# B-R-P/NMSLIB-ZIG

Measured on AMD Instinct MI355X. Metric: queries/sec @ recall@10, 1M x 128-D L2, batch=1024; HBM GB/s vs peak, higher is better.
Workload: dtype f16+f32

## Files before the change

nmslib_zig_amd/csrc/brute.cpp:

```cpp
#include <algorithm>
#include <cmath>
#include <cstdlib>
#include <cstring>

#include "engine.hpp"
#include "l1_quant.hpp"

namespace gfxknn {

void BruteDense::release() {
    have_bf16 = false;
    have_l1 = false;
    l1_u8.release();
    l1_cols.release();
    bf_hi.release();
    bf_lo.release();
    f16_hi.release();
    auxp.release();
    auxp16.release();
}

size_t BruteDense::bytes() const {
    size_t total = 0;
    for (const DevBuf* b : {&rows_i8, &auxh, &rows_sel, &mean, &bf_hi, &bf_lo, &auxp, &f16_hi, &auxp16, &l1_u8, &l1_cols}) total += b->bytes();
// ... 228 lines not shown
    auto fast_ws = [&](const BfFastWsBytes& need) {
        BfFastWs ws{};
        ws.top8 = b.ws_top8.ensure(need.top8);
        ws.thr = b.ws_thr.ensure(need.thr);
        ws.list = static_cast<uint32_t*>(b.ws_list.ensure(need.list));
        ws.list_cnt = static_cast<int*>(b.ws_listcnt.ensure(need.list_cnt));
        ws.fb.cand = static_cast<unsigned long long*>(ws_cand_.ensure(need.cand));
        ws.fb.cnt = static_cast<int*>(ws_cnt_.ensure(need.cnt));
        if (need.flags_fb) ws.flags_fb = static_cast<int*>(b.ws_flags.ensure(need.flags_fb));
        if (need.queries) ws.queries = b.ws_f32_q.ensure(need.queries);
        return ws;
    };
    if (is_u8()) {
        const BfU8Fast f = bf_u8_fast_plan((int)d_n_, (int)nq, (int)k);
        if (f.use) {
            ws_qpad_.ensure((size_t)f.qpad * 128);
            const BfFastWs ws = fast_ws(bf_fast_ws_bytes(f));
            const BfU8Rows rows{d_rows_.as<uint8_t>(), b.rows_i8.as<uint8_t>(), d_aux_.as<int32_t>(), b.auxh.as<int32_t>(), (int)d_n_};
            hip_check(launch_bf_u8_fast(f, (int)nq, (int)k, rows, static_cast<const uint8_t*>(d_queries), ws_qpad_.as<uint8_t>(),
                                        ws, out, prof_pair(), stream),
                      "bf_u8_fast");
            last_path = 3;
            fast_flags_ = ws.tile_fail(f);
            fast_nqt_ = f.nqt;
            fast_has_precise_ = false;
            return;
        }
    }
    const BfF32Rows rows{d_rows_.as<float>(), b.centred ? b.rows_sel.as<float>() : d_rows_.as<float>(), d_aux_.as<float>(),
                         (int)d_n_, dim_eff, d_n_ ? ldb_ : f32_row_stride(dim_eff), b.bmax};
    BfF32Queries q{};
    if (!is_u8() && b.have_bf16) {
        const BfF32Fast f = bf_f32_fast_plan((int)d_n_, dim_eff, (int)nq, (int)k, space_, b.centred);
        if (f.use) {
            const int ldb = ldb_;
            q.padded = static_cast<float*>(ws_qpad_.ensure((size_t)f.qpad * ldb * 4));
            q.sel = q.padded;
            q.scale_q = b.f16_scale_q;
            if (b.centred) {
                hip_check(launch_pad_rows(d_queries, (int)nq, dim_eff, q.padded, f.qpad, ldb, 4, stream), "pad queries");
                ws_qsel_.ensure((size_t)f.qpad * ldb * 4);
                hip_check(launch_center_rows(q.padded, b.mean.as<float>(), f.qpad, (int)nq, ldb, dim_eff, ws_qsel_.as<float>(),
                                             stream),
                          "centre queries");
                q.sel = ws_qsel_.as<float>();
            } else {
                q.raw = static_cast<const float*>(d_queries);
            }
            if (f.cosc) {
                ws_qaux_.ensure((size_t)f.qpad * 16);
                b.ws_qaug.ensure((size_t)f.qpad * f.dp * 4);
                q.centred = ws_qsel_.as<float>();
                q.qaux_cosc = ws_qaux_.as<float>();
                hip_check(launch_query_aux_cosc(q.padded, q.centred, f.qpad, ldb, dim_eff, b.mu_norm, ws_qaux_.as<float>(), stream),
                          "query aux");
                hip_check(launch_query_aug_cosc(q.centred, q.qaux_cosc, (int)nq, f.qpad, ldb, dim_eff, b.cosc_lambda,
                                                b.ws_qaug.as<float>(), f.dp, stream),
                          "augmented queries");
                q.sel = b.ws_qaug.as<float>();
                q.sel_ld = f.dp;
            }
            const BfFastWs ws = fast_ws(bf_fast_ws_bytes(f));
            hip_check(launch_bf_f32_fast(f, space_, (int)nq, (int)k, rows, b.tiles(f.dp, f.cosc), q, ws, out, prof_pair(), stream),
                      "bf_f32_fast");
            last_path = 1;
            fast_flags_ = ws.tile_fail(f);
            fast_nqt_ = f.nqt;
            fast_has_precise_ = true;
            return;
        }
    }
    if (space_ == SP_L1 && b.have_l1) {
        const char* env = getenv("NMSLIB_GPU_L1_FAST");
        const BfL1Fast f = bf_l1_fast_plan((int)d_n_, dim_eff, (int)nq, (int)k);
        if (f.use && !(env && atoi(env) == 0)) {
            ws_qpad_.ensure((size_t)f.qpad * ldb_ * 4);
            BfL1Ws ws{};
            ws.qt = static_cast<uint32_t*>(b.ws_l1_qt.ensure((size_t)f.d4 * f.qpad * 4));
            ws.xe = static_cast<double*>(b.ws_l1_xe.ensure((size_t)f.qpad * 16));
            ws.cand.cand = static_cast<unsigned long long*>(b.ws_l1_cand.ensure((size_t)f.qpad * f.nsplit * f.kprime * 8));
            ws.cand.cnt = static_cast<int*>(b.ws_l1_cnt.ensure((size_t)f.qpad * f.nsplit * 4));
            ws.flags = static_cast<int*>(b.ws_flags.ensure((size_t)f.nqt * 4 + 64));
            ws.fb.cand = static_cast<unsigned long long*>(ws_cand_.ensure(bf_cand_elems(f.fallback) * 8));
            ws.fb.cnt = static_cast<int*>(ws_cnt_.ensure(bf_cnt_elems(f.fallback) * 4));
            const float* cols = b.l1_cols.as<float>();
            const BfL1Rows copy{b.l1_u8.as<uint32_t>(), cols, cols + dim_, cols + 2 * dim_, b.l1_step};
            hip_check(launch_bf_l1_fast(f, (int)nq, (int)k, rows, copy, static_cast<const float*>(d_queries), ws_qpad_.as<float>(),
                                        ws, out, prof_pair(), stream),
                      "bf_l1_fast");
            last_path = 6;
            fast_flags_ = ws.flags;
            fast_nqt_ = f.nqt;
            fast_has_precise_ = false;
            return;
        }
    }
    last_path = is_u8() ? 2 : 0;
    BfPlan p = bf_make_plan((int)d_n_, dim_eff, (int)nq, (int)k, is_u8());
    if (d_n_ == 0) p.ldb = is_u8() ? 128 : f32_row_stride(dim_eff);
    const int elem = is_u8() ? 1 : 4;
    ws_qpad_.ensure((size_t)p.qpad * p.ldb * elem);
    const BfCand c{static_cast<unsigned long long*>(ws_cand_.ensure(bf_cand_elems(p) * 8)),
                   static_cast<int*>(ws_cnt_.ensure(bf_cnt_elems(p) * 4))};
    hip_check(launch_pad_rows(d_queries, (int)nq, dim_eff, ws_qpad_.ptr(), p.qpad, p.ldb, elem, stream), "pad queries");
    q.padded = ws_qpad_.as<float>();
    q.sel = q.padded;
    if (b.centred) {
        ws_qsel_.ensure((size_t)p.qpad * p.ldb * 4);
        hip_check(launch_center_rows(q.padded, b.mean.as<float>(), p.qpad, (int)nq, p.ldb, dim_eff, ws_qsel_.as<float>(), stream),
                  "centre queries");
        q.sel = ws_qsel_.as<float>();
        if (space_ != SP_L2) {
            ws_qaux_.ensure((size_t)p.qpad * 16);
            hip_check(launch_query_aux_cosc(q.padded, q.sel, p.qpad, p.ldb, dim_eff, b.mu_norm, ws_qaux_.as<float>(), stream),
// ... 24 lines not shown
```

nmslib_zig_amd/csrc/engine.cpp:

```cpp
#include "engine.hpp"
#include "f16_pack.hpp"

#include <algorithm>
#include <chrono>
#include <cmath>
#include <cstring>
#include <fstream>
#include <set>
#include <sstream>
#include <thread>

namespace gfxknn {

using clk = std::chrono::steady_clock;

void hip_check(hipError_t e, const char* what) {
    if (e == hipSuccess) return;
    std::string msg = std::string(what) + ": " + hipGetErrorString(e);
    (void)hipGetLastError();
    throw EngineError(e == hipErrorOutOfMemory ? Err::OutOfMemory : Err::Runtime, msg);
}

ParamSet::ParamSet(const std::vector<std::string>& desc) {
    std::set<std::string> seen;
// ... 269 lines not shown
    ids_.clear();
    rows_f32_.clear();
    rows_u8_.clear();
    sp_ptr_.assign(1, 0);
    sp_ids_.clear();
    sp_vals_.clear();
    st_ptr_.assign(1, 0);
    st_bytes_.clear();
    st_words_.clear();
    st_bits_ = -1;
    graph_ = HostGraph();
    graph_rows_.clear();
    loaded_graph_ = false;
    graph_builder_ = 0;
    created_ = false;
    dirty_ = true;
    graph_dirty_ = true;
    d_n_ = 0;
    shards_.clear();
    dim_ = 0;
    brute_ = BruteDense();
    last_path = 0;
    fast_flags_ = nullptr;
    fast_nqt_ = 0;
    hnsw_fix_valid_ = false;
    have_counters_ = false;
    d_rows16_.release();
    rows16_failed_ = false;
    rows_f16_index_ = rows_f16_ = false;
    rerank_ = 0;
}

size_t Engine::memory_usage() const {
    if (!created_) return 0;
    if (sparse_)
        return ids_.size() * 16 + sp_ids_.size() * sizeof(SparseElem) + hbm_bytes();
    if (str_space_)
        return ids_.size() * 16 + (space_ == SP_LEVEN ? st_bytes_.size() : ids_.size() * (ham_words() + 1) * 4) +
               hbm_bytes();
    size_t total = ids_.size() * (16 + stored_row_bytes());
    total += ids_.size() * dim_ * sizeof(float);
    return total + rows16_bytes();
}

size_t Engine::rows16_bytes() const {
    size_t b = d_rows16_.bytes();
// ... 747 lines not shown
    }
    for (size_t q0 = 0; q0 < nq; q0 += slice) {
        const size_t m = std::min(slice, nq - q0);
        ctr_off_ = q0;
        const void* qs = static_cast<const char*>(d_queries) + q0 * qbytes;
        int32_t* cnt = d_cnt ? d_cnt + q0 : nullptr;
        if (method_ == Method::Brute) knn_brute(qs, m, k, d_ids + q0 * k, d_dists + q0 * k, cnt, stream);
        else knn_hnsw(qs, m, k, d_ids + q0 * k, d_dists + q0 * k, cnt, stream);
    }
}

void Engine::fast_tile_counts(size_t* tiles, size_t* precise, size_t* fallback) {
    *tiles = *precise = *fallback = 0;
    if (!shards_.empty()) {
        shards_[0]->fast_tile_counts(tiles, precise, fallback);
        return;
    }
    if ((last_path != 1 && last_path != 3 && last_path != 6) || !fast_flags_ || fast_nqt_ <= 0) return;
    std::vector<int> h((size_t)fast_nqt_ * 2, 0);
    hip_check(hipSetDevice(device_), "hipSetDevice");
    hip_check(hipStreamSynchronize(last_stream_ ? last_stream_ : stream_), "stats");
    hip_check(hipMemcpy(h.data(), fast_flags_, (size_t)fast_nqt_ * (fast_has_precise_ ? 2 : 1) * sizeof(int), hipMemcpyDeviceToHost),
              "stats flags");
    *tiles = (size_t)fast_nqt_;
    for (int i = 0; i < fast_nqt_; ++i) {
        *fallback += h[i] != 0;
        if (fast_has_precise_) *precise += h[(size_t)fast_nqt_ + i] != 0;
    }
}

size_t Engine::hnsw_redone() {
    if (!shards_.empty()) return shards_[0]->hnsw_redone();
    if ((last_path != 4 && last_path != 5) || !hnsw_fix_valid_) return 0;
    int32_t v = 0;
    hip_check(hipSetDevice(device_), "hipSetDevice");
    hip_check(hipStreamSynchronize(last_stream_ ? last_stream_ : stream_), "stats");
    hip_check(hipMemcpy(&v, ws_fix_.ptr(), 4, hipMemcpyDeviceToHost), "stats redo count");
    return (size_t)v;
}

HnswOut Engine::hnsw_out(int32_t* d_ids, float* d_dists, int32_t* d_cnt, size_t nq) {
    if (!d_cnt) {
        ws_outcnt_.ensure(nq * 4);
        d_cnt = ws_outcnt_.as<int32_t>();
    }
    return {d_ids, d_dists, d_cnt, ws_ndc_.as<int32_t>() + ctr_off_, ws_hops_.as<int32_t>() + ctr_off_,
// ... 602 lines not shown
```

nmslib_zig_amd/csrc/engine.hpp:

```cpp
#pragma once
#include <hip/hip_runtime_api.h>

#include <cstdint>
#include <functional>
#include <map>
#include <memory>
#include <mutex>
#include <stdexcept>
#include <string>
#include <utility>
#include <vector>

#include "kernels/kernels.hpp"

namespace gfxknn {

enum class Err : int {
    InvalidArgument = 2,
    OutOfMemory = 3,
    SpaceIncompatible = 5,
    QueryTooLarge = 6,
    IndexBuildFailed = 8,
    QueryExecutionFailed = 9,
    DataIO = 10,
// ... 171 lines not shown
    float pair_distance(size_t p1, size_t p2);
    size_t range_host(const void* query, size_t elem_count, double radius, size_t capacity, int32_t* ids, float* dists);
    bool is_brute() const { return method_ == Method::Brute; }

    void save(const std::string& path, bool save_data);
    static std::unique_ptr<Engine> load(const std::string& path, int data_type, int dist_type, bool load_data);

    size_t thread_pool_size = 0;
    size_t memory_usage() const;

    const int32_t* last_ndc() const { return have_counters_ ? ws_ndc_.as<int32_t>() : nullptr; }
    const int32_t* last_hops() const { return have_counters_ ? ws_hops_.as<int32_t>() : nullptr; }
    const int32_t* last_hops_up() const { return have_counters_ ? ws_hops_up_.as<int32_t>() : nullptr; }

    void set_profiling(bool on) { prof_ = on; }
    void collect_profile(double* total_ms, uint64_t* launches);

    double upload_seconds = 0, build_seconds = 0;
    int last_path = 0;
    size_t rows16_bytes() const;
    const int* fast_flags_ = nullptr;
    int fast_nqt_ = 0;
    bool fast_has_precise_ = false;
    void fast_tile_counts(size_t* tiles, size_t* precise, size_t* fallback);
    size_t hnsw_redone();
    hipStream_t last_stream_ = nullptr;
    bool hnsw_fix_valid_ = false;
    size_t hbm_bytes() const;

    std::mutex mu;

    size_t shard_count() const { return shards_.size(); }
    int graph_builder() const { return shards_.empty() ? graph_builder_ : shards_[0]->graph_builder_; }

   private:
    const float* rows_f32() const { return parent_ ? parent_->rows_f32_.data() + view_lo_ * dim_ : rows_f32_.data(); }
    const uint8_t* rows_u8() const { return parent_ ? parent_->rows_u8_.data() + view_lo_ * 128 : rows_u8_.data(); }
    int resolve_shards() const;
    void finalize_sharded(int nshards);
    void knn_sharded(const void* d_queries, size_t nq, size_t elem_count, size_t k, int32_t* d_ids, float* d_dists,
                     int32_t* d_cnt, hipStream_t stream);
    std::vector<std::unique_ptr<Engine>> shards_;
    std::vector<hipEvent_t> shard_events_;
    hipEvent_t shard_ready_ = nullptr;
    const Engine* parent_ = nullptr;
    size_t view_lo_ = 0, view_n_ = 0;
// ... 130 lines not shown
```

nmslib_zig_amd/csrc/kernels/bf_kernels.hip:

```cpp
#include <cstdio>
#include <type_traits>
#include <vector>
#include <cstdlib>

#include "common_dev.hpp"
#include "kernels.hpp"

namespace gfxknn {

enum BfMode : int { BF_L2 = 0, BF_DOT = 1, BF_COS = 2, BF_L1 = 3, BF_LINF = 4, BF_COSC = 5, BF_L2D = 6 };

struct BfArgs {
    const float* base;
    const float* aux;
    const float* qaux;
    int aux_stride;
    const float* queries;
    u64* cand;
    int* cand_cnt;
    uint32_t* gthr;
    uint32_t* gq;
    int xj, xm;
    int n, ldb, nqt, nsplit, rows_per_split, kprime, cap;
    int kcs;
// ... 144 lines not shown
    const int per = nsplit >> 2;
    const u64* r64 = reinterpret_cast<const u64*>(row) + h * per;
    for (int i = 0; i < per; ++i) {
        const u64 w = __hip_atomic_load(r64 + i, __ATOMIC_RELAXED, __HIP_MEMORY_SCOPE_AGENT);
        const int s0 = 2 * (h * per + i);
        ins(s0 == split ? pu : (uint32_t)w);
        ins(s0 + 1 == split ? pu : (uint32_t)(w >> 32));
    }
    uint32_t o[8];
#pragma unroll
    for (int i = 0; i < 8; ++i) o[i] = __shfl_xor(tm[i], 32, 64);
#pragma unroll
    for (int i = 0; i < 8; ++i) ins(o[i]);
    uint32_t t = tm[0];
#pragma unroll
    for (int i = 1; i < 8; ++i) t = (i == xm - 1) ? tm[i] : t;
    return t;
}

__device__ long long g_bf_clk[2];
__device__ long long g_bf_trace[2048][3];

template <int MODE, bool FULL, bool ONE>
__global__ __launch_bounds__(256, 2) void bf_select_f32_kernel(BfArgs a) {
    extern __shared__ __attribute__((aligned(16))) char smem[];
    const int tid = threadIdx.x, lane = tid & 63, wave = tid >> 6;
    const long long clk_c0 = __builtin_readcyclecounter(), clk_r0 = wall_clock64();
    const int h = lane >> 5, l31 = lane & 31;

    const int b = blockIdx.x;
    const int xcd = b & 7, rest = b >> 3;
    const int qt = rest % a.nqt;
    const int split = (rest / a.nqt) * 8 + xcd;
    if (split >= a.nsplit) return;
    if (a.tile_fail && a.tile_fail[qt / a.fail_group] == 0) return;

    constexpr bool kDirect = (MODE == BF_L1 || MODE == BF_LINF || MODE == BF_L2D);
    constexpr bool kDelay = !kDirect;
    constexpr bool kCosC = (MODE == BF_COSC);
    constexpr int kAuxN = kCosC ? 3 : 1;
    constexpr bool kAux = (MODE == BF_L2 || MODE == BF_COS || kCosC);

    const int kcs = FULL ? BF_KC : a.kcs;
    const int lds_stride = kcs + 4;
    float* tile = reinterpret_cast<float*>(smem);
    float* auxs = tile + 2 * BF_BN * lds_stride;
    u64* scratch = reinterpret_cast<u64*>(auxs + 4 * BF_BN * 3) + (size_t)wave * a.cap;

    const int qidx = qt * BF_TQ + wave * 32 + l31;
    const int half = a.cap >> 1;
    u64* candq = a.cand + ((size_t)qidx * a.nsplit + split) * a.cap + (size_t)h * half;
    int mycnt = 0;
    u64* wave_cand = a.cand + ((size_t)(qt * BF_TQ + wave * 32) * a.nsplit + split) * a.cap;
    const size_t qstride = (size_t)a.nsplit * a.cap;
    const bool use_top8 = a.kprime <= 16;
    const bool track8 = use_top8 || a.xj > 0;
    float t8[8];
#pragma unroll
// ... 344 lines not shown
                    if (a.xj > 0 && !(a.dbg & (256 | 512))) exchange_counted();
                    finish_stage(true);
                }
            }
        }
        if ((!FULL || kDirect) && have_next && !((a.dbg & 2) && step > 0)) write_lds(step + 1);
        flush_pending();
        if (lastc && !(a.dbg & 256)) {
            if (a.xj > 0 && !(a.dbg & 512)) {
                if ((stage & (stage + 1)) == 0 || (stage & 31) == 31) exchange_counted();
            } else if ((stage & xmask) == xmask) {
                exchange_thr();
            }
        }
        if (!(a.dbg & 8)) __syncthreads();
    }
    if (kDelay && nstages > 0 && !skip_epi) {
        check_block(accY, 1, nstages - 1);
        if (a.xj > 0 && !(a.dbg & (256 | 512))) exchange_counted();
        if (!(a.dbg & 16)) finish_stage(true);
    }
    if (h == 0) a.cand_cnt[(size_t)qidx * a.nsplit + split] = mycnt;
    if ((a.dbg & 1024) && tid == 0) {
        if (blockIdx.x == 0) {
            g_bf_clk[0] = __builtin_readcyclecounter() - clk_c0;
            g_bf_clk[1] = wall_clock64() - clk_r0;
        }
        if (blockIdx.x < 2048) {
            g_bf_trace[blockIdx.x][0] = clk_r0;
            g_bf_trace[blockIdx.x][1] = wall_clock64();
            g_bf_trace[blockIdx.x][2] = __builtin_amdgcn_s_getreg((4 << 0) | (0 << 6) | (31 << 11));
        }
    }
}

struct BfArgsU8 {
    const uint8_t* base_i8;
    const int32_t* aux;
    const uint8_t* queries;
    u64* cand;
    int* cand_cnt;
    uint32_t* gq;
    int xj, xm;
    int n, nqt, nsplit, rows_per_split, kprime, cap;
    int dbg;
    int tile_stride;
    const int* tile_fail;
    int fail_group;
};

typedef const __attribute__((address_space(1))) void* gptr_t;
typedef __attribute__((address_space(3))) void* lptr_t;

__global__ __launch_bounds__(256, 2) void bf_select_u8_kernel(BfArgsU8 a) {
    extern __shared__ __attribute__((aligned(16))) char smem[];
    const int tid = threadIdx.x, lane = tid & 63, wave = tid >> 6;
// ... 1777 lines not shown
        atomicMax(out_bits + 3, __float_as_uint(mh));
    }
}

struct RerankArgs {
    const void* base;
    const void* queries;
    const u64* cand;
    const int* cand_cnt;
    const int32_t* ext_ids;
    int32_t* out_ids;
    float* out_dists;
    int32_t* out_cnt;
    int space, dim, ldb, k, nsplit, cap, kprime, p2max;
    const int* tile_fail;
    int fail_queries;
    int* verify_flags;
    int verify_queries;
    const float* queries_sel;
    float bmax;
    float eps_rel;
};

__global__ __launch_bounds__(256) void bf_rerank_kernel(RerankArgs a) {
    extern __shared__ __attribute__((aligned(16))) char smem[];
    u64* keys = reinterpret_cast<u64*>(smem);
    int* offs = reinterpret_cast<int*>(keys + a.p2max);
    const int q = blockIdx.x, tid = threadIdx.x, lane = tid & 63, wave = tid >> 6;
    if (a.tile_fail && a.tile_fail[q / a.fail_queries] == 0) return;

    if (tid == 0) {
        int o = 0;
        for (int s = 0; s < a.nsplit; ++s) {
            offs[s] = o;
            int c = a.cand_cnt[(size_t)q * a.nsplit + s];
            o += c < a.kprime ? c : a.kprime;
        }
        offs[a.nsplit] = o;
    }
    __syncthreads();
    const int total = offs[a.nsplit];
    __shared__ uint32_t s_kth;
    const bool verify = a.verify_flags != nullptr && a.space == SP_L2 && total >= a.kprime;
    if (tid == 0) s_kth = 0xffffffffu;
    for (int idx = tid; idx < a.nsplit * a.kprime; idx += blockDim.x) {
        const int s = idx / a.kprime, i = idx - s * a.kprime;
        const int c = offs[s + 1] - offs[s];
        if (i < c) keys[offs[s] + i] = a.cand[((size_t)q * a.nsplit + s) * a.cap + i];
    }
    __syncthreads();
    if (verify) {
        for (int i = tid; i < total; i += blockDim.x) {
// ... 60 lines not shown
        }
        a.out_ids[(size_t)q * a.k + i] = id;
        a.out_dists[(size_t)q * a.k + i] = d;
    }
    if (tid == 0 && a.out_cnt) a.out_cnt[q] = found;
    if (verify && found > 0) {
        __shared__ float s_qn2v;
        if (tid < 64) {
            const float* qs = a.queries_sel + (size_t)q * a.ldb;
            float ss = 0.f;
            for (int d = tid; d < a.dim; d += 64) ss = fmaf(qs[d], qs[d], ss);
            ss = wave_sum(ss);
            if (tid == 0) s_qn2v = ss;
        }
        __syncthreads();
        if (tid == 0) {
            const float qn2 = s_qn2v, qn = sqrtf(qn2);
            const float kth = ord_f32(s_kth);
            const float dk = ord_f32((uint32_t)(keys[found - 1] >> 32));
            const float e = a.eps_rel * (qn * a.bmax + 0.5f * a.bmax * a.bmax);
            const float floor_d2 = qn2 - 2.0f * kth - 2.0f * e - 2e-6f * (qn2 + fabsf(kth));
            if (!(dk * dk <= floor_d2)) atomicOr(&a.verify_flags[q / a.verify_queries], 1);
        }
    }
}

__global__ void row_aux_f32_kernel(const float* base, int n, int ldb, int dim, int space, float* aux) {
    const int lane = threadIdx.x & 63;
    const int row = blockIdx.x * (blockDim.x >> 6) + (threadIdx.x >> 6);
    if (row >= n) return;
    const float* p = base + (size_t)row * ldb;
    float s = 0.f;
    for (int d = lane; d < dim; d += 64) s = fmaf(p[d], p[d], s);
    s = wave_sum(s);
    if (lane == 0) {
        float v = 0.f;
        if (space == SP_L2) v = -0.5f * s;
        else if (space == SP_COSINE || space == SP_ANGULAR)
            v = (s < 1.17549435e-38f * 2.0f) ? 0.f : 1.0f / sqrtf(s);
        aux[row] = v;
    }
}

__global__ void prepare_u8_kernel(const uint8_t* base, int n, int n_pad, uint8_t* rows_i8, int32_t* aux, int32_t* auxh) {
    const int lane = threadIdx.x & 63;
    const int row = blockIdx.x * (blockDim.x >> 6) + (threadIdx.x >> 6);
// ... 391 lines not shown
    a.queries = q;
    a.cand = c.cand;
    a.cand_cnt = c.cnt;
    a.tile_fail = gate.flags;
    a.fail_group = gate.tiles;
    a.gthr = gthr;
    a.gq = gthr + p.qpad;
    a.xj = p.xj;
    a.xm = p.xm;
    a.n = p.n;
    a.ldb = p.ldb;
    a.nqt = p.nqt;
    a.nsplit = p.nsplit;
    a.rows_per_split = p.rows_per_split;
    a.kprime = p.kprime;
    a.cap = p.cap;
    a.kcs = p.ldb < BF_KC ? p.ldb : BF_KC;
    a.nchunks = (p.ldb + BF_KC - 1) / BF_KC;
    static const int dbg = getenv("NMSLIB_GPU_DEBUG") ? atoi(getenv("NMSLIB_GPU_DEBUG")) : 0;
    a.dbg = dbg;
    return a;
}

static hipError_t select_f32(const BfPlan& p, int space, const float* base, const float* aux, const float* queries_padded,
                             const float* qaux_cosc, const BfCand& c, const BfGate& gate, hipStream_t s, bool cleared) {
    uint32_t* gthr = reinterpret_cast<uint32_t*>(c.cnt + (size_t)p.qpad * p.nsplit);
    if (!cleared) {
        hipError_t me = hipMemsetAsync(gthr, 0, ((size_t)p.qpad + (size_t)p.qpad * p.nsplit) * 4, s);
        if (me != hipSuccess) return me;
    }
    BfArgs a = make_args(p, base, aux, queries_padded, c, gate, gthr);
    switch (space) {
        case SP_L2: return launch_select_mode<BF_L2>(p, a, s);
        case SP_NEGDOT: return launch_select_mode<BF_DOT>(p, a, s);
        case SP_COSINE:
        case SP_ANGULAR:
            if (qaux_cosc) {
                a.qaux = qaux_cosc;
                a.aux_stride = p.n;
                return launch_select_mode<BF_COSC>(p, a, s);
            }
            return launch_select_mode<BF_COS>(p, a, s);
        default: return hipErrorInvalidValue;
    }
}

hipError_t launch_bf_select_direct_f32(const BfPlan& p, int space, const float* base, const float* queries_padded,
                                       const BfCand& c, const BfGate& gate, hipStream_t s, bool cleared_second_region) {
    const size_t gwords = (size_t)p.qpad + (size_t)p.qpad * p.nsplit;
    uint32_t* gthr = reinterpret_cast<uint32_t*>(c.cnt + (size_t)p.qpad * p.nsplit);
    if (cleared_second_region) {
        gthr += gwords;
    } else {
        hipError_t me = hipMemsetAsync(gthr, 0, gwords * 4, s);
        if (me != hipSuccess) return me;
    }
    BfArgs a = make_args(p, base, nullptr, queries_padded, c, gate, gthr);
    if (space == SP_L1) return launch_select_mode<BF_L1>(p, a, s);
    if (space == SP_LINF) return launch_select_mode<BF_LINF>(p, a, s);
    if (space == SP_L2) return launch_select_mode<BF_L2D>(p, a, s);
    return hipErrorInvalidValue;
}

hipError_t launch_bf_select_u8(const BfPlan& p, const uint8_t* base_i8, const int32_t* aux, const uint8_t* queries_padded,
                               const BfCand& c, const BfGate& gate, hipStream_t s, bool cleared) {
// ... 10 lines not shown
    a.nqt = p.nqt;
    a.nsplit = p.nsplit;
    a.rows_per_split = p.rows_per_split;
    a.kprime = p.kprime;
    a.cap = p.cap;
    uint32_t* gthr = reinterpret_cast<uint32_t*>(c.cnt + (size_t)p.qpad * p.nsplit);
    a.gq = gthr + p.qpad;
    a.xj = p.xj;
    a.xm = p.xm;
    static const int dbg = getenv("NMSLIB_GPU_DEBUG") ? atoi(getenv("NMSLIB_GPU_DEBUG")) : 0;
    a.dbg = dbg;
    if (!cleared) {
        hipError_t me = hipMemsetAsync(gthr, 0, ((size_t)p.qpad + (size_t)p.qpad * p.nsplit) * 4, s);
        if (me != hipSuccess) return me;
    }
    hipError_t e = hipFuncSetAttribute(reinterpret_cast<const void*>(bf_select_u8_kernel),
                                       hipFuncAttributeMaxDynamicSharedMemorySize, (int)p.lds_select);
    if (e != hipSuccess) return e;
    const int grid = 8 * p.nqt * (p.nsplit / 8);
    hipLaunchKernelGGL(bf_select_u8_kernel, dim3(grid), dim3(256), p.lds_select, s, a);
    return hipGetLastError();
}

hipError_t launch_bf_rerank(const BfPlan& p, int space, int dim, int k, const void* base, const void* queries_padded,
                            const BfCand& c, const BfGate& gate, const BfVerify& verify, const BfOut& out, hipStream_t s) {
    RerankArgs a{};
    a.verify_flags = verify.flags;
    a.verify_queries = BF_TQ;
    a.queries_sel = verify.queries_sel;
    a.bmax = verify.bmax;
    a.eps_rel = 1.5f * (float)(dim + 2) * 5.9604645e-8f;
    a.tile_fail = gate.flags;
    a.fail_queries = gate.tiles * BF_TQ;
    a.base = base;
    a.queries = queries_padded;
    a.cand = c.cand;
    a.cand_cnt = c.cnt;
    a.ext_ids = out.ext_ids;
    a.out_ids = out.ids;
    a.out_dists = out.dists;
    a.out_cnt = out.cnt;
    a.space = space;
    a.dim = dim;
    a.ldb = p.ldb;
    a.k = k;
    a.nsplit = p.nsplit;
    a.cap = p.cap;
    a.kprime = p.kprime;
    a.p2max = p.p2max;
    hipError_t e = hipFuncSetAttribute(reinterpret_cast<const void*>(bf_rerank_kernel),
                                       hipFuncAttributeMaxDynamicSharedMemorySize, (int)p.lds_rerank);
    if (e != hipSuccess) return e;
    hipLaunchKernelGGL(bf_rerank_kernel, dim3(p.nq), dim3(256), p.lds_rerank, s, a);
    return hipGetLastError();
}

hipError_t launch_bf_adaptive_f32(const BfPlan& p, int space, int k, const BfF32Rows& rows, const BfF32Queries& q,
                                  const BfCand& c, int* flags, const BfGate& gate, const BfOut& out, hipStream_t s,
                                  bool cleared) {
    hipError_t e = select_f32(p, space, rows.sel, rows.aux, q.sel, q.qaux_cosc, c, gate, s, cleared);
    if (e != hipSuccess) return e;
    const bool verify = space == SP_L2 && flags != nullptr && rows.bmax > 0.f;
    if (!verify) return launch_bf_rerank(p, space, rows.dim, k, rows.orig, q.padded, c, gate, BfVerify{}, out, s);
    if (!cleared) {
        e = hipMemsetAsync(flags, 0, (size_t)p.nqt * 4, s);
        if (e != hipSuccess) return e;
    }
    e = launch_bf_rerank(p, space, rows.dim, k, rows.orig, q.padded, c, gate, BfVerify{flags, q.sel, rows.bmax}, out, s);
    if (e != hipSuccess) return e;
    const BfGate failed{flags, 1};
    e = launch_bf_select_direct_f32(p, SP_L2, rows.orig, q.padded, c, failed, s, cleared);
    if (e != hipSuccess) return e;
    return launch_bf_rerank(p, space, rows.dim, k, rows.orig, q.padded, c, failed, BfVerify{}, out, s);
}

BfU8Fast bf_u8_fast_plan(int n, int nq, int k) {
    BfU8Fast f{};
    f.use = (n >= 65536 && nq >= 512 && k <= 256);
    if (const char* e = getenv("NMSLIB_GPU_U8_FAST")) f.use = f.use && atoi(e) != 0;
    if (!f.use) return f;
    f.qg = nq >= 2048 ? 4 : 2;
    const int tq = BF_TQ * f.qg;
    f.qpad = (nq + tq - 1) / tq * tq;
    f.nqt = f.qpad / tq;
    f.stride = 8;
    if (const char* e = getenv("NMSLIB_GPU_U8_STRIDE")) f.stride = atoi(e) > 0 ? atoi(e) : 8;
    const double kf = (double)k / f.stride;
    f.r = (int)(1.6 * kf + 3.0 * sqrt(kf) + 3.0 + 0.999);
    const int tiles_all = (n + BF_BN - 1) / BF_BN;
    int ns = (512 + f.nqt - 1) / f.nqt;
    if (ns > tiles_all / 16) ns = tiles_all / 16;
    if (ns > 256) ns = 256;
    ns = (ns + 7) / 8 * 8;
    if (ns < 8) ns = 8;
    while ((tiles_all + ns - 1) / ns > 32768) ns += 8;
    f.nsplit = ns;
// ... 295 lines not shown
hipError_t launch_bf_f32_fast(const BfF32Fast& f, int space, int nq, int k, const BfF32Rows& rows, const BfF32Tiles& tiles,
                              const BfF32Queries& q, const BfFastWs& ws, const BfOut& out, const BfScanEvents& ev,
                              hipStream_t s) {
    const int sdim = f.cosc ? f.sel_dim : rows.dim, sld = f.cosc ? q.sel_ld : rows.ldb;
    float* top8 = static_cast<float*>(ws.top8);
    float* thr = static_cast<float*>(ws.thr);
    float* thr1 = ws.thr1(f);
    int* tile_fail = ws.tile_fail(f);
    int* precise = ws.precise(f);
    void* q_hi = ws.q_tile(f, BfFastWs::Q_HI);
    void* q_lo = ws.q_tile(f, BfFastWs::Q_LO);
    void* q_h16 = ws.q_tile(f, BfFastWs::Q_H16);
    hipError_t e;
    {
        const BfPlan& fb = f.fallback;
        uint32_t* gthr = reinterpret_cast<uint32_t*>(ws.fb.cnt + (size_t)fb.qpad * fb.nsplit);
        const size_t gwords = 2 * ((size_t)fb.qpad + (size_t)fb.qpad * fb.nsplit);
        size_t work = (size_t)f.qpad * f.dp > gwords ? (size_t)f.qpad * f.dp : gwords;
        size_t grid = (work + 255) / 256;
        if (grid > 2048) grid = 2048;
        hipLaunchKernelGGL(bf_f32_prep_kernel, dim3((unsigned)grid), dim3(256), 0, s, q.raw, nq, sdim, q.sel, f.qpad,
                           sld, q.raw ? q.padded : nullptr, f.kch > 1 ? nullptr : static_cast<__bf16*>(q_hi),
                           f.kch > 1 ? nullptr : static_cast<__bf16*>(q_lo),
                           tile_fail, 2 * f.nqt, ws.flags_fb, fb.nqt, gthr, gwords, f.dp, static_cast<_Float16*>(q_h16), q.scale_q);
        e = hipGetLastError();
        if (e != hipSuccess) return e;
    }
    auto scan = [&](const BfScanF32Args& sa, bool sample, int terms, int grid) -> hipError_t {
        const size_t lds = terms == 1 ? f.lds_scan1 : f.lds_scan;
        if (f.mode == 0) return launch_scan_f32_mode<SC_L2>(sa, sample, terms, f.qg, grid, lds, s, f.kch);
        if (f.mode == 1) return launch_scan_f32_mode<SC_DOT>(sa, sample, terms, f.qg, grid, lds, s, f.kch);
        return launch_scan_f32_mode<SC_COS>(sa, sample, terms, f.qg, grid, lds, s, f.kch);
    };
    BfScanF32Args a{};
    a.base_hi = static_cast<const __bf16*>(tiles.hi);
    a.base_lo = static_cast<const __bf16*>(tiles.lo);
    a.auxp = tiles.auxp;
    a.q_hi = static_cast<const __bf16*>(q_hi);
    a.q_lo = static_cast<const __bf16*>(q_lo);
    a.base_h16 = tiles.h16;
    {
        static const int prio = getenv("NMSLIB_GPU_BF16_PRIO") ? atoi(getenv("NMSLIB_GPU_BF16_PRIO")) : 0;
        a.prio_half = prio;
    }
    a.q_h16 = q_h16;
    a.auxp16 = tiles.auxp16;
    a.n = rows.n;
// ... 72 lines not shown
    r.thr1 = thr1;
    r.precise = precise;
    r.list_m_off = ws.list_m_off(f);
    r.bmax = tiles.bmax;
    r.bres = tiles.bres;
    static const int dbg = getenv("NMSLIB_GPU_DEBUG") ? atoi(getenv("NMSLIB_GPU_DEBUG")) : 0;
    static unsigned long long* d_prof = nullptr;
    if (dbg & 4096) {
        if (!d_prof) (void)hipMalloc(&d_prof, 16 * 8);
        (void)hipMemsetAsync(d_prof, 0, 16 * 8, s);
        r.prof = d_prof;
    }
    e = hipFuncSetAttribute(reinterpret_cast<const void*>(bf_rerank_f32_list_kernel),
                            hipFuncAttributeMaxDynamicSharedMemorySize, (int)f.lds_rerank);
    if (e != hipSuccess) return e;
    hipLaunchKernelGGL(bf_rerank_f32_list_kernel, dim3(nq), dim3(256), f.lds_rerank, s, r);
    e = hipGetLastError();
    if (e != hipSuccess) return e;
    if (dbg & 4096) dump_rerank_list_clocks(d_prof, s);
    if (dbg & 2048) dump_f32_fast_checksums(f, ws, s);
    BfF32Queries fq = q;
    fq.sel = f.cosc ? q.centred : q.sel;
    fq.qaux_cosc = f.cosc ? q.qaux_cosc : nullptr;
    return launch_bf_adaptive_f32(f.fallback, space, k, rows, fq, ws.fb, ws.flags_fb, BfGate{tile_fail, f.tq / 128}, out, s,
                                  true);
}

hipError_t launch_row_aux_f32(const float* base, int n, int ldb, int dim, int space, float* aux,
                              hipStream_t s) {
    if (n == 0) return hipSuccess;
    hipLaunchKernelGGL(row_aux_f32_kernel, dim3((n + 3) / 4), dim3(256), 0, s, base, n, ldb, dim, space, aux);
    return hipGetLastError();
}
hipError_t launch_prepare_u8(const uint8_t* base, int n, uint8_t* rows_i8, int32_t* aux, int32_t* auxh, hipStream_t s) {
    const int n_pad = bf_u8_rows_padded(n);
    hipLaunchKernelGGL(prepare_u8_kernel, dim3((n_pad + 3) / 4), dim3(256), 0, s, base, n, n_pad, rows_i8, aux, auxh);
    return hipGetLastError();
}
hipError_t launch_pad_rows(const void* src, int rows, int dim, void* dst, int rows_pad, int ld,
                           int elem_bytes, hipStream_t s) {
    const size_t total = (size_t)rows_pad * ld * elem_bytes;
    if (total == 0) return hipSuccess;
    int grid = (int)((total + 255) / 256);
    if (grid > 4096) grid = 4096;
    hipLaunchKernelGGL(pad_rows_kernel, dim3(grid), dim3(256), 0, s, (const uint8_t*)src, rows,
                       dim * elem_bytes, (uint8_t*)dst, rows_pad, ld * elem_bytes);
    return hipGetLastError();
}
// ... 79 lines not shown
```

nmslib_zig_amd/csrc/kernels/kernels.hpp:

```cpp
#pragma once
#include <hip/hip_runtime_api.h>
#include <stddef.h>
#include <stdint.h>

#include <utility>

namespace gfxknn {

enum SpaceCode : int {
    SP_L2 = 0,
    SP_L1 = 1,
    SP_LINF = 2,
    SP_COSINE = 3,
    SP_ANGULAR = 4,
    SP_NEGDOT = 5,
    SP_L2SQR_SIFT = 6,
    SP_L2SQR = 7,
    SP_NORMCOS = 8,
    SP_QNORM_NEGDOT = 9,
    SP_LEVEN = 10,
    SP_BIT_HAMMING = 11,
    SP_KLDIV = 12,
    SP_KLDIV_RQ = 13,
    SP_KLDIVGEN = 14,
// ... 74 lines not shown
    const float* sel;
    const float* centred;
    const float* qaux_cosc;
    int sel_ld;
    float scale_q;
};
struct BfU8Rows {
    const uint8_t *orig, *i8;
    const int32_t *aux, *auxh;
    int n;
};
using BfScanEvents = std::pair<hipEvent_t, hipEvent_t>;

hipError_t launch_bf_select_u8(const BfPlan& p, const uint8_t* base_i8, const int32_t* aux, const uint8_t* queries_padded,
                               const BfCand& c, const BfGate& gate, hipStream_t s, bool cleared = false);
hipError_t launch_bf_select_direct_f32(const BfPlan& p, int space, const float* base, const float* queries_padded,
                                       const BfCand& c, const BfGate& gate, hipStream_t s,
                                       bool cleared_second_region = false);
hipError_t launch_bf_rerank(const BfPlan& p, int space, int dim, int k, const void* base, const void* queries_padded,
                            const BfCand& c, const BfGate& gate, const BfVerify& verify, const BfOut& out, hipStream_t s);
hipError_t launch_bf_adaptive_f32(const BfPlan& p, int space, int k, const BfF32Rows& rows, const BfF32Queries& q,
                                  const BfCand& c, int* flags, const BfGate& gate, const BfOut& out, hipStream_t s,
                                  bool cleared = false);

struct BfU8Fast {
    bool use;
    int qg;
    int qpad, nqt;
    int stride, r;
    int nsplit, tps, caph;
    int p2max;
    size_t lds_scan, lds_thr, lds_rerank;
    int s_nsplit, s_tps;
    BfPlan fallback;
};
BfU8Fast bf_u8_fast_plan(int n, int nq, int k);

struct BfF32Fast {
    bool use;
    int mode;
    int qg;
    bool cosc;
    int sel_dim;
    int kch;
    int dp;
    int tq;
// ... 16 lines not shown
    return {(size_t)f.qpad * f.s_nsplit * 2 * 8 * 4, (size_t)f.qpad * 4 + (size_t)f.nqt * 4 + 64, lists * f.caph * 4, lists * 4,
            bf_cand_elems(f.fallback) * 8, bf_cnt_elems(f.fallback) * 4, 0, 0};
}
inline BfFastWsBytes bf_fast_ws_bytes(const BfF32Fast& f) {
    const size_t lists = (size_t)f.qpad * f.nsplit * 2;
    return {(size_t)f.qpad * f.s_nsplit * 2 * 8 * 4, (size_t)f.qpad * 8 + (size_t)f.nqt * 8 + 64, 2 * lists * f.caph * 4, lists * 4,
            bf_cand_elems(f.fallback) * 8, bf_cnt_elems(f.fallback) * 4, (size_t)f.fallback.nqt * 4 + 64,
            (size_t)f.qpad * f.dp * 2 * 3};
}
struct BfFastWs {
    void* top8;
    void* thr;
    uint32_t* list;
    int* list_cnt;
    BfCand fb;
    int* flags_fb;
    void* queries;

    size_t list_m_off(const BfF32Fast& f) const { return (size_t)f.qpad * f.caph * f.nsplit * 2; }
    int* tile_fail(const BfU8Fast& f) const { return static_cast<int*>(thr) + f.qpad; }
    float* thr1(const BfF32Fast& f) const { return static_cast<float*>(thr) + f.qpad; }
    int* tile_fail(const BfF32Fast& f) const { return reinterpret_cast<int*>(thr1(f) + f.qpad); }
    int* precise(const BfF32Fast& f) const { return tile_fail(f) + f.nqt; }
    enum QueryTile { Q_HI = 0, Q_LO = 1, Q_H16 = 2 };
    void* q_tile(const BfF32Fast& f, QueryTile t) const { return static_cast<char*>(queries) + (size_t)t * f.qpad * f.dp * 2; }
};

hipError_t launch_bf_u8_fast(const BfU8Fast& f, int nq, int k, const BfU8Rows& rows, const uint8_t* queries_raw,
                             uint8_t* queries_padded, const BfFastWs& ws, const BfOut& out, const BfScanEvents& ev,
                             hipStream_t s);

inline int bf_f32_rows_padded(int n) { return (n + BF_BN - 1) / BF_BN * BF_BN + BF_BN; }
hipError_t launch_row_maxnorm(const float* rows, int n, int ld, int dim, bool relative_residual, float* out, hipStream_t s,
                              float scale16 = 0.f);
struct BfF32Tiles {
    void *hi, *lo;
    float* auxp;
    void* h16;
    float* auxp16;
    float scale, bres16;
    int dp;
    float bmax, bres;
};
struct BfSplitSrc {
    const float* rows;
    int n, n_pad, ld, cols;
};
hipError_t launch_split_bf16(const BfSplitSrc& src, const float* aux, float aux_pad, float aux16_mul, const BfF32Tiles& dst,
                             hipStream_t s);
// ... 284 lines not shown
```

Baseline: 3.054 million.

## Replace multi-kernel fallback chain with a single persistent ticketed tail kernel

```diff
diff --git a/nmslib_zig_amd/csrc/brute.cpp b/nmslib_zig_amd/csrc/brute.cpp
--- a/nmslib_zig_amd/csrc/brute.cpp
+++ b/nmslib_zig_amd/csrc/brute.cpp
@@ -274,6 +274,7 @@
                       "bf_u8_fast");
             last_path = 3;
             fast_flags_ = ws.tile_fail(f);
+            fast_tail_stuck_ = nullptr;
             fast_nqt_ = f.nqt;
             fast_has_precise_ = false;
             return;
@@ -317,6 +318,7 @@
                       "bf_f32_fast");
             last_path = 1;
             fast_flags_ = ws.tile_fail(f);
+            fast_tail_stuck_ = ws.tail_words(f) + BfFastWs::TAIL_STUCK;
             fast_nqt_ = f.nqt;
             fast_has_precise_ = true;
             return;
@@ -342,6 +344,7 @@
                       "bf_l1_fast");
             last_path = 6;
             fast_flags_ = ws.flags;
+            fast_tail_stuck_ = nullptr;
             fast_nqt_ = f.nqt;
             fast_has_precise_ = false;
             return;
diff --git a/nmslib_zig_amd/csrc/engine.cpp b/nmslib_zig_amd/csrc/engine.cpp
--- a/nmslib_zig_amd/csrc/engine.cpp
+++ b/nmslib_zig_amd/csrc/engine.cpp
@@ -315,6 +315,7 @@
     brute_ = BruteDense();
     last_path = 0;
     fast_flags_ = nullptr;
+    fast_tail_stuck_ = nullptr;
     fast_nqt_ = 0;
     hnsw_fix_valid_ = false;
     have_counters_ = false;
@@ -1108,6 +1109,13 @@
     hip_check(hipStreamSynchronize(last_stream_ ? last_stream_ : stream_), "stats");
     hip_check(hipMemcpy(h.data(), fast_flags_, (size_t)fast_nqt_ * (fast_has_precise_ ? 2 : 1) * sizeof(int), hipMemcpyDeviceToHost),
               "stats flags");
+    if (last_path == 1 && fast_tail_stuck_) {
+        int stuck = 0;
+        hip_check(hipMemcpy(&stuck, fast_tail_stuck_, sizeof(int), hipMemcpyDeviceToHost), "stats tail word");
+        if (stuck != 0)
+            throw EngineError(Err::QueryExecutionFailed, "brute force: a wait of the fallback tail kernel ran out; the results of "
+                                                         "the last batch are incomplete");
+    }
     *tiles = (size_t)fast_nqt_;
     for (int i = 0; i < fast_nqt_; ++i) {
         *fallback += h[i] != 0;
diff --git a/nmslib_zig_amd/csrc/engine.hpp b/nmslib_zig_amd/csrc/engine.hpp
--- a/nmslib_zig_amd/csrc/engine.hpp
+++ b/nmslib_zig_amd/csrc/engine.hpp
@@ -217,6 +217,7 @@
     const int* fast_flags_ = nullptr;
     int fast_nqt_ = 0;
     bool fast_has_precise_ = false;
+    const int* fast_tail_stuck_ = nullptr;
     void fast_tile_counts(size_t* tiles, size_t* precise, size_t* fallback);
     size_t hnsw_redone();
     hipStream_t last_stream_ = nullptr;
diff --git a/nmslib_zig_amd/csrc/kernels/bf_kernels.hip b/nmslib_zig_amd/csrc/kernels/bf_kernels.hip
--- a/nmslib_zig_amd/csrc/kernels/bf_kernels.hip
+++ b/nmslib_zig_amd/csrc/kernels/bf_kernels.hip
@@ -190,18 +190,16 @@
 __device__ long long g_bf_trace[2048][3];
 
 template <int MODE, bool FULL, bool ONE>
-__global__ __launch_bounds__(256, 2) void bf_select_f32_kernel(BfArgs a) {
-    extern __shared__ __attribute__((aligned(16))) char smem[];
+__device__ __forceinline__ void bf_select_f32_block(const BfArgs& a, const int b, char* smem) {
     const int tid = threadIdx.x, lane = tid & 63, wave = tid >> 6;
     const long long clk_c0 = __builtin_readcyclecounter(), clk_r0 = wall_clock64();
     const int h = lane >> 5, l31 = lane & 31;
 
-    const int b = blockIdx.x;
     const int xcd = b & 7, rest = b >> 3;
     const int qt = rest % a.nqt;
     const int split = (rest / a.nqt) * 8 + xcd;
     if (split >= a.nsplit) return;
-    if (a.tile_fail && a.tile_fail[qt / a.fail_group] == 0) return;
+    if (a.tile_fail && __hip_atomic_load(&a.tile_fail[qt / a.fail_group], __ATOMIC_RELAXED, __HIP_MEMORY_SCOPE_AGENT) == 0) return;
 
     constexpr bool kDirect = (MODE == BF_L1 || MODE == BF_LINF || MODE == BF_L2D);
     constexpr bool kDelay = !kDirect;
@@ -592,16 +590,22 @@
     }
     if (h == 0) a.cand_cnt[(size_t)qidx * a.nsplit + split] = mycnt;
     if ((a.dbg & 1024) && tid == 0) {
-        if (blockIdx.x == 0) {
+        if (b == 0) {
             g_bf_clk[0] = __builtin_readcyclecounter() - clk_c0;
             g_bf_clk[1] = wall_clock64() - clk_r0;
         }
-        if (blockIdx.x < 2048) {
-            g_bf_trace[blockIdx.x][0] = clk_r0;
-            g_bf_trace[blockIdx.x][1] = wall_clock64();
-            g_bf_trace[blockIdx.x][2] = __builtin_amdgcn_s_getreg((4 << 0) | (0 << 6) | (31 << 11));
-        }
-    }
+        if (b < 2048) {
+            g_bf_trace[b][0] = clk_r0;
+            g_bf_trace[b][1] = wall_clock64();
+            g_bf_trace[b][2] = __builtin_amdgcn_s_getreg((4 << 0) | (0 << 6) | (31 << 11));
+        }
+    }
+}
+
+template <int MODE, bool FULL, bool ONE>
+__global__ __launch_bounds__(256, 2) void bf_select_f32_kernel(BfArgs a) {
+    extern __shared__ __attribute__((aligned(16))) char smem[];
+    bf_select_f32_block<MODE, FULL, ONE>(a, blockIdx.x, smem);
 }
 
 struct BfArgsU8 {
@@ -2425,12 +2429,11 @@
     float eps_rel;
 };
 
-__global__ __launch_bounds__(256) void bf_rerank_kernel(RerankArgs a) {
-    extern __shared__ __attribute__((aligned(16))) char smem[];
+__device__ __forceinline__ void bf_rerank_block(const RerankArgs& a, const int q, char* smem) {
     u64* keys = reinterpret_cast<u64*>(smem);
     int* offs = reinterpret_cast<int*>(keys + a.p2max);
-    const int q = blockIdx.x, tid = threadIdx.x, lane = tid & 63, wave = tid >> 6;
-    if (a.tile_fail && a.tile_fail[q / a.fail_queries] == 0) return;
+    const int tid = threadIdx.x, lane = tid & 63, wave = tid >> 6;
+    if (a.tile_fail && __hip_atomic_load(&a.tile_fail[q / a.fail_queries], __ATOMIC_RELAXED, __HIP_MEMORY_SCOPE_AGENT) == 0) return;
 
     if (tid == 0) {
         int o = 0;
@@ -2537,6 +2540,79 @@
             const float floor_d2 = qn2 - 2.0f * kth - 2.0f * e - 2e-6f * (qn2 + fabsf(kth));
             if (!(dk * dk <= floor_d2)) atomicOr(&a.verify_flags[q / a.verify_queries], 1);
         }
+    }
+}
+
+__global__ __launch_bounds__(256) void bf_rerank_kernel(RerankArgs a) {
+    extern __shared__ __attribute__((aligned(16))) char smem[];
+    bf_rerank_block(a, blockIdx.x, smem);
+}
+
+struct BfTailArgs {
+    BfArgs sel, sel_exact;
+    RerankArgs rr, rr_exact;
+    BfPlan plan;
+    int has_verify;
+    const int* tile_fail;
+    int n_fail;
+    int* words;
+};
+constexpr int kTailMaxPolls = 1 << 18;
+
+template <int MODE, bool FULL, bool ONE>
+__global__ __launch_bounds__(256, 2) void bf_fallback_tail_kernel(BfTailArgs a) {
+    extern __shared__ __attribute__((aligned(16))) char smem[];
+    __shared__ int s_tail[2];
+    const int tid = threadIdx.x;
+    {
+        int any = 0;
+        for (int i = 0; i < a.n_fail; ++i) any |= a.tile_fail[i];
+        if (any == 0) return;
+    }
+    int* const done = a.words + BfFastWs::TAIL_DONE;
+    int* const stuck = a.words + BfFastWs::TAIL_STUCK;
+    for (;;) {
+        if (tid == 0)
+            s_tail[0] = __hip_atomic_fetch_add(a.words + BfFastWs::TAIL_TICKET, 1, __ATOMIC_RELAXED, __HIP_MEMORY_SCOPE_AGENT);
+        __syncthreads();
+        const BfTailItem it = bf_tail_item(a.plan, a.has_verify != 0, __builtin_amdgcn_readfirstlane(s_tail[0]));
+        if (it.phase == 0) return;
+        if (it.phase > 1) {
+            if (tid == 0) {
+                const int need = it.count[it.phase - 1];
+                int ok = 1, last = -1, polls = 0;
+                for (;;) {
+                    const int v = __hip_atomic_load(done + it.phase - 2, __ATOMIC_ACQUIRE, __HIP_MEMORY_SCOPE_AGENT);
+                    if (v >= need) break;
+                    if (__hip_atomic_load(stuck, __ATOMIC_RELAXED, __HIP_MEMORY_SCOPE_AGENT) != 0) {
+                        ok = 0;
+                        break;
+                    }
+                    if (v != last) {
+                        last = v;
+                        polls = 0;
+                    } else if (++polls >= kTailMaxPolls) {
+                        __hip_atomic_store(stuck, 1, __ATOMIC_RELAXED, __HIP_MEMORY_SCOPE_AGENT);
+                        ok = 0;
+                        break;
+                    }
+                    __builtin_amdgcn_s_sleep(32);
+                }
+                s_tail[1] = ok;
+            }
+            __syncthreads();
+            if (__builtin_amdgcn_readfirstlane(s_tail[1]) == 0) return;
+            __builtin_amdgcn_fence(__ATOMIC_ACQUIRE, "agent");
+        }
+        if (it.phase == 1) bf_select_f32_block<MODE, FULL, ONE>(a.sel, it.index, smem);
+        else if (it.phase == 2) bf_rerank_block(a.rr, it.index, smem);
+        if constexpr (MODE == BF_L2) {
+            if (it.phase == 3) bf_select_f32_block<BF_L2D, false, false>(a.sel_exact, it.index, smem);
+            else if (it.phase == 4) bf_rerank_block(a.rr_exact, it.index, smem);
+        }
+        __builtin_amdgcn_fence(__ATOMIC_RELEASE, "agent");
+        __syncthreads();
+        if (tid == 0) __hip_atomic_fetch_add(done + it.phase - 1, 1, __ATOMIC_RELEASE, __HIP_MEMORY_SCOPE_AGENT);
     }
 }
 
@@ -2974,25 +3050,37 @@
     return a;
 }
 
-static hipError_t select_f32(const BfPlan& p, int space, const float* base, const float* aux, const float* queries_padded,
-                             const float* qaux_cosc, const BfCand& c, const BfGate& gate, hipStream_t s, bool cleared) {
+static int select_f32_args(const BfPlan& p, int space, const float* base, const float* aux, const float* queries_padded,
+                           const float* qaux_cosc, const BfCand& c, const BfGate& gate, BfArgs* a) {
     uint32_t* gthr = reinterpret_cast<uint32_t*>(c.cnt + (size_t)p.qpad * p.nsplit);
-    if (!cleared) {
-        hipError_t me = hipMemsetAsync(gthr, 0, ((size_t)p.qpad + (size_t)p.qpad * p.nsplit) * 4, s);
-        if (me != hipSuccess) return me;
-    }
-    BfArgs a = make_args(p, base, aux, queries_padded, c, gate, gthr);
+    *a = make_args(p, base, aux, queries_padded, c, gate, gthr);
     switch (space) {
-        case SP_L2: return launch_select_mode<BF_L2>(p, a, s);
-        case SP_NEGDOT: return launch_select_mode<BF_DOT>(p, a, s);
+        case SP_L2: return BF_L2;
+        case SP_NEGDOT: return BF_DOT;
         case SP_COSINE:
         case SP_ANGULAR:
             if (qaux_cosc) {
-                a.qaux = qaux_cosc;
-                a.aux_stride = p.n;
-                return launch_select_mode<BF_COSC>(p, a, s);
-            }
-            return launch_select_mode<BF_COS>(p, a, s);
+                a->qaux = qaux_cosc;
+                a->aux_stride = p.n;
+                return BF_COSC;
+            }
+            return BF_COS;
+        default: return -1;
+    }
+}
+static hipError_t select_f32(const BfPlan& p, int space, const float* base, const float* aux, const float* queries_padded,
+                             const float* qaux_cosc, const BfCand& c, const BfGate& gate, hipStream_t s, bool cleared) {
+    BfArgs a;
+    const int mode = select_f32_args(p, space, base, aux, queries_padded, qaux_cosc, c, gate, &a);
+    if (!cleared) {
+        hipError_t me = hipMemsetAsync(a.gthr, 0, ((size_t)p.qpad + (size_t)p.qpad * p.nsplit) * 4, s);
+        if (me != hipSuccess) return me;
+    }
+    switch (mode) {
+        case BF_L2: return launch_select_mode<BF_L2>(p, a, s);
+        case BF_DOT: return launch_select_mode<BF_DOT>(p, a, s);
+        case BF_COSC: return launch_select_mode<BF_COSC>(p, a, s);
+        case BF_COS: return launch_select_mode<BF_COS>(p, a, s);
         default: return hipErrorInvalidValue;
     }
 }
@@ -3049,8 +3137,8 @@
     return hipGetLastError();
 }
 
-hipError_t launch_bf_rerank(const BfPlan& p, int space, int dim, int k, const void* base, const void* queries_padded,
-                            const BfCand& c, const BfGate& gate, const BfVerify& verify, const BfOut& out, hipStream_t s) {
+static RerankArgs make_rerank_args(const BfPlan& p, int space, int dim, int k, const void* base, const void* queries_padded,
+                                   const BfCand& c, const BfGate& gate, const BfVerify& verify, const BfOut& out) {
     RerankArgs a{};
     a.verify_flags = verify.flags;
     a.verify_queries = BF_TQ;
@@ -3075,6 +3163,12 @@
     a.cap = p.cap;
     a.kprime = p.kprime;
     a.p2max = p.p2max;
+    return a;
+}
+
+hipError_t launch_bf_rerank(const BfPlan& p, int space, int dim, int k, const void* base, const void* queries_padded,
+                            const BfCand& c, const BfGate& gate, const BfVerify& verify, const BfOut& out, hipStream_t s) {
+    const RerankArgs a = make_rerank_args(p, space, dim, k, base, queries_padded, c, gate, verify, out);
     hipError_t e = hipFuncSetAttribute(reinterpret_cast<const void*>(bf_rerank_kernel),
                                        hipFuncAttributeMaxDynamicSharedMemorySize, (int)p.lds_rerank);
     if (e != hipSuccess) return e;
@@ -3099,6 +3193,69 @@
     e = launch_bf_select_direct_f32(p, SP_L2, rows.orig, q.padded, c, failed, s, cleared);
     if (e != hipSuccess) return e;
     return launch_bf_rerank(p, space, rows.dim, k, rows.orig, q.padded, c, failed, BfVerify{}, out, s);
+}
+
+static int bf_cu_count() {
+    static int cus[64] = {};
+    int dev = 0;
+    if (hipGetDevice(&dev) != hipSuccess || dev < 0 || dev >= 64) return 256;
+    if (cus[dev] == 0) {
+        int v = 0;
+        if (hipDeviceGetAttribute(&v, hipDeviceAttributeMultiprocessorCount, dev) != hipSuccess || v <= 0) v = 256;
+        cus[dev] = v;
+    }
+    return cus[dev];
+}
+template <int MODE>
+static hipError_t launch_tail_mode(const BfPlan& p, const BfTailArgs& a, int grid, size_t lds, hipStream_t s) {
+    auto go = [&](auto kern) -> hipError_t {
+        hipError_t e = hipFuncSetAttribute(reinterpret_cast<const void*>(kern), hipFuncAttributeMaxDynamicSharedMemorySize, (int)lds);
+        if (e != hipSuccess) return e;
+        hipLaunchKernelGGL(kern, dim3(grid), dim3(256), lds, s, a);
+        return hipGetLastError();
+    };
+#ifdef BF_FAST_COMPILE
+    if (MODE == BF_L2 && p.ldb == BF_KC) return go(bf_fallback_tail_kernel<BF_L2, true, true>);
+    return hipErrorInvalidValue;
+#else
+    if (p.ldb == BF_KC) return go(bf_fallback_tail_kernel<MODE, true, true>);
+    if (p.ldb % BF_KC == 0) return go(bf_fallback_tail_kernel<MODE, true, false>);
+    return go(bf_fallback_tail_kernel<MODE, false, false>);
+#endif
+}
+hipError_t launch_bf_fallback_tail(const BfPlan& p, int space, int k, const BfF32Rows& rows, const BfF32Queries& q,
+                                   const BfCand& c, int* flags, int* tail_words, const BfGate& gate, const BfOut& out,
+                                   hipStream_t s) {
+    if (!gate.flags || !flags || !tail_words) return hipErrorInvalidValue;
+    BfTailArgs a{};
+    const int mode = select_f32_args(p, space, rows.sel, rows.aux, q.sel, q.qaux_cosc, c, gate, &a.sel);
+    const bool verify = space == SP_L2 && rows.bmax > 0.f;
+    a.rr = make_rerank_args(p, space, rows.dim, k, rows.orig, q.padded, c, gate,
+                            verify ? BfVerify{flags, q.sel, rows.bmax} : BfVerify{}, out);
+    if (verify) {
+        const BfGate failed{flags, 1};
+        const size_t gwords = (size_t)p.qpad + (size_t)p.qpad * p.nsplit;
+        uint32_t* gthr = reinterpret_cast<uint32_t*>(c.cnt + (size_t)p.qpad * p.nsplit) + gwords;
+        a.sel_exact = make_args(p, rows.orig, nullptr, q.padded, c, failed, gthr);
+        a.rr_exact = make_rerank_args(p, space, rows.dim, k, rows.orig, q.padded, c, failed, BfVerify{}, out);
+    }
+    a.plan = p;
+    a.has_verify = verify ? 1 : 0;
+    a.tile_fail = gate.flags;
+    a.n_fail = (p.nqt + gate.tiles - 1) / gate.tiles;
+    a.words = tail_words;
+    const int total = bf_tail_item(p, verify, 0).total;
+    const int slots = 2 * bf_cu_count();
+    const int grid = total < slots ? total : slots;
+    if (grid <= 0) return hipSuccess;
+    const size_t lds = p.lds_select > p.lds_rerank ? p.lds_select : p.lds_rerank;
+    switch (mode) {
+        case BF_L2: return launch_tail_mode<BF_L2>(p, a, grid, lds, s);
+        case BF_DOT: return launch_tail_mode<BF_DOT>(p, a, grid, lds, s);
+        case BF_COSC: return launch_tail_mode<BF_COSC>(p, a, grid, lds, s);
+        case BF_COS: return launch_tail_mode<BF_COS>(p, a, grid, lds, s);
+        default: return hipErrorInvalidValue;
+    }
 }
 
 BfU8Fast bf_u8_fast_plan(int n, int nq, int k) {
@@ -3440,7 +3597,8 @@
         hipLaunchKernelGGL(bf_f32_prep_kernel, dim3((unsigned)grid), dim3(256), 0, s, q.raw, nq, sdim, q.sel, f.qpad,
                            sld, q.raw ? q.padded : nullptr, f.kch > 1 ? nullptr : static_cast<__bf16*>(q_hi),
                            f.kch > 1 ? nullptr : static_cast<__bf16*>(q_lo),
-                           tile_fail, 2 * f.nqt, ws.flags_fb, fb.nqt, gthr, gwords, f.dp, static_cast<_Float16*>(q_h16), q.scale_q);
+                           tile_fail, 2 * f.nqt, ws.flags_fb, fb.nqt + BfFastWs::TAIL_WORDS, gthr, gwords, f.dp,
+                           static_cast<_Float16*>(q_h16), q.scale_q);
         e = hipGetLastError();
         if (e != hipSuccess) return e;
     }
@@ -3559,8 +3717,11 @@
     BfF32Queries fq = q;
     fq.sel = f.cosc ? q.centred : q.sel;
     fq.qaux_cosc = f.cosc ? q.qaux_cosc : nullptr;
-    return launch_bf_adaptive_f32(f.fallback, space, k, rows, fq, ws.fb, ws.flags_fb, BfGate{tile_fail, f.tq / 128}, out, s,
-                                  true);
+    const BfGate failed{tile_fail, f.tq / 128};
+    const char* tail = getenv("NMSLIB_GPU_BF_TAIL");
+    if (tail && atoi(tail) == 0)
+        return launch_bf_adaptive_f32(f.fallback, space, k, rows, fq, ws.fb, ws.flags_fb, failed, out, s, true);
+    return launch_bf_fallback_tail(f.fallback, space, k, rows, fq, ws.fb, ws.flags_fb, ws.tail_words(f), failed, out, s);
 }
 
 hipError_t launch_row_aux_f32(const float* base, int n, int ldb, int dim, int space, float* aux,
diff --git a/nmslib_zig_amd/csrc/kernels/kernels.hpp b/nmslib_zig_amd/csrc/kernels/kernels.hpp
--- a/nmslib_zig_amd/csrc/kernels/kernels.hpp
+++ b/nmslib_zig_amd/csrc/kernels/kernels.hpp
@@ -120,6 +120,35 @@
 hipError_t launch_bf_adaptive_f32(const BfPlan& p, int space, int k, const BfF32Rows& rows, const BfF32Queries& q,
                                   const BfCand& c, int* flags, const BfGate& gate, const BfOut& out, hipStream_t s,
                                   bool cleared = false);
+hipError_t launch_bf_fallback_tail(const BfPlan& p, int space, int k, const BfF32Rows& rows, const BfF32Queries& q,
+                                   const BfCand& c, int* flags, int* tail_words, const BfGate& gate, const BfOut& out,
+                                   hipStream_t s);
+
+constexpr int BF_TAIL_PHASES = 4;
+struct BfTailItem {
+    int phase;
+    int index;
+    int count[BF_TAIL_PHASES + 1];
+    int total;
+};
+__host__ __device__ inline BfTailItem bf_tail_item(const BfPlan& p, bool has_verify, int ticket) {
+    BfTailItem it{};
+    const int sel = 8 * p.nqt * (p.nsplit / 8);
+    it.count[1] = sel;
+    it.count[2] = p.nq;
+    it.count[3] = has_verify ? sel : 0;
+    it.count[4] = has_verify ? p.nq : 0;
+    int first = 0;
+    for (int ph = 1; ph <= BF_TAIL_PHASES; ++ph) {
+        if (it.phase == 0 && ticket >= first && ticket - first < it.count[ph]) {
+            it.phase = ph;
+            it.index = ticket - first;
+        }
+        first += it.count[ph];
+    }
+    it.total = first;
+    return it;
+}
 
 struct BfU8Fast {
     bool use;
@@ -182,9 +211,13 @@
     float* thr1(const BfF32Fast& f) const { return static_cast<float*>(thr) + f.qpad; }
     int* tile_fail(const BfF32Fast& f) const { return reinterpret_cast<int*>(thr1(f) + f.qpad); }
     int* precise(const BfF32Fast& f) const { return tile_fail(f) + f.nqt; }
+    enum TailWord { TAIL_TICKET = 0, TAIL_DONE = 1, TAIL_STUCK = TAIL_DONE + BF_TAIL_PHASES, TAIL_WORDS };
+    int* tail_words(const BfF32Fast& f) const { return flags_fb + f.fallback.nqt; }
     enum QueryTile { Q_HI = 0, Q_LO = 1, Q_H16 = 2 };
     void* q_tile(const BfF32Fast& f, QueryTile t) const { return static_cast<char*>(queries) + (size_t)t * f.qpad * f.dp * 2; }
 };
+
+static_assert(BfFastWs::TAIL_WORDS * 4 <= 64, "the tail words live in the 64 spare bytes of the flags_fb block");
 
 hipError_t launch_bf_u8_fast(const BfU8Fast& f, int nq, int k, const BfU8Rows& rows, const uint8_t* queries_raw,
                              uint8_t* queries_padded, const BfFastWs& ws, const BfOut& out, const BfScanEvents& ev,
```

Result: no change. 3.057 million, median of 5 (+0.1%).
